# mmailhos/vectorlite

Measured on AMD Instinct MI355X. Metric: flat-cosine QPS @ N=10M dim=384 k=10; achieved HBM GB/s vs peak, higher is better.
Workload: dtype f32; 1 GPU; flat cosine single-query search, N=10000000, dim=384, k=10; rows=10000000, dim=384, k=10, metric=cosine, parallelism=1 GPU

## Files before the change

### vectorlite_amd/csrc/device_common.hpp

```cpp
#pragma once

#include <hip/hip_runtime.h>
#include <math.h>
#include <stdint.h>

#include "kernels.hpp"

namespace vl {
namespace dev {

typedef float f32x4 __attribute__((ext_vector_type(4)));

constexpr int WAVE = 64;

__device__ __forceinline__ int lane_id() { return threadIdx.x & (WAVE - 1); }

template <typename K>
__device__ __forceinline__ bool better(K ka, uint32_t pa, K kb, uint32_t pb)
{
    return ka > kb || (ka == kb && pa < pb);
}

__device__ __forceinline__ int wave_shr1_dw(int v) { return __builtin_amdgcn_update_dpp(v, v, 0x138, 0xF, 0xF, false); }
__device__ __forceinline__ float wave_shr1(float v) { return __int_as_float(wave_shr1_dw(__float_as_int(v))); }
// ... 99 lines not shown
    return rust_as_u64(__longlong_as_double((long long)key));
}


template <typename K>
__device__ __forceinline__ K neg_inf();
template <>
__device__ __forceinline__ float neg_inf<float>() { return -INFINITY; }
template <>
__device__ __forceinline__ double neg_inf<double>() { return -(double)INFINITY; }

template <typename K>
struct TopList {
    K key;
    uint32_t pos;
    K thr_key;
    uint32_t thr_pos;

    __device__ __forceinline__ void init()
    {
        key = neg_inf<K>();
        pos = POS_SENTINEL;
        asm volatile("" : "+v"(key));
        thr_key = read_lane(key, WAVE - 1);
        thr_pos = POS_SENTINEL;
    }

    __device__ __forceinline__ void insert(K k, uint32_t p)
    {
        const unsigned long long ahead = __ballot(better<K>(key, pos, k, p));
        const int idx = __popcll(ahead);
        const K upk = wave_shr1(key);
        const uint32_t upp = wave_shr1(pos);
        const int lane = lane_id();
        if (lane == idx) {
            key = k;
            pos = p;
        } else if (lane > idx) {
            key = upk;
            pos = upp;
        }
        thr_key = read_lane(key, WAVE - 1);
        thr_pos = read_lane(pos, WAVE - 1);
    }

    __device__ __forceinline__ void offer(K k, uint32_t p, bool active)
    {
        unsigned long long m = __ballot(active && better<K>(k, p, thr_key, thr_pos));
        while (m) {
            const int src = __builtin_amdgcn_readfirstlane(__ffsll((long long)m) - 1);
            m &= m - 1;
            insert(read_lane(k, src), read_lane(p, src));
        }
    }

    __device__ __forceinline__ void merge_reversed(K ok, uint32_t op)
    {
        if (better<K>(ok, op, key, pos)) {
            key = ok;
            pos = op;
        }
        const int lane = lane_id();
#pragma unroll
        for (int o = WAVE / 2; o >= 1; o >>= 1) {
            const K k2 = __shfl_xor(key, o);
            const uint32_t p2 = __shfl_xor(pos, o);
            const bool lower = (lane & o) == 0;
            const bool other_better = better<K>(k2, p2, key, pos);
            if (lower == other_better) {
                key = k2;
                pos = p2;
            }
        }
        thr_key = read_lane(key, WAVE - 1);
        thr_pos = read_lane(pos, WAVE - 1);
    }
};

template <typename K>
__device__ __forceinline__ void sort64_reversed(K& key, uint32_t& pos)
{
    const int lane = lane_id();
#pragma unroll
    for (int k = 2; k <= WAVE; k <<= 1) {
#pragma unroll
        for (int j = k >> 1; j >= 1; j >>= 1) {
            const K k2 = __shfl_xor(key, j);
            const uint32_t p2 = __shfl_xor(pos, j);
            const bool up = (lane & k) == 0;
            const bool keep_worse = ((lane & j) == 0) == up;
            const bool other_worse = better<K>(key, pos, k2, p2);
            if (keep_worse == other_worse) {
                key = k2;
                pos = p2;
            }
        }
    }
}

template <typename K, typename C, int NW>
__device__ __forceinline__ void block_merge(TopList<K>& L, C* sh )
{
    const int lane = lane_id();
    const int wave = threadIdx.x >> 6;
    sh[wave * WAVE + lane].key = L.key;
    sh[wave * WAVE + lane].pos = L.pos;
    __syncthreads();
#pragma unroll
    for (int s = NW / 2; s >= 1; s >>= 1) {
        if (wave < s) {
            const C o = sh[(wave + s) * WAVE + (WAVE - 1 - lane)];
            L.merge_reversed(o.key, o.pos);
            sh[wave * WAVE + lane].key = L.key;
            sh[wave * WAVE + lane].pos = L.pos;
        }
        __syncthreads();
    }
}

template <typename K, typename C>
__device__ __forceinline__ void block_merge_n(TopList<K>& L, C* sh, int active)
{
    const int lane = lane_id();
    const int wave = threadIdx.x >> 6;
    int top = 1;
    while (top < active) top <<= 1;
    if (wave < top) {
        sh[wave * WAVE + lane].key = L.key;
        sh[wave * WAVE + lane].pos = L.pos;
    }
    __syncthreads();
    for (int s = top / 2; s >= 1; s >>= 1) {
        if (wave < s) {
            const C o = sh[(wave + s) * WAVE + (WAVE - 1 - lane)];
            L.merge_reversed(o.key, o.pos);
            sh[wave * WAVE + lane].key = L.key;
            sh[wave * WAVE + lane].pos = L.pos;
        }
        __syncthreads();
    }
}

template <typename C>
__device__ __forceinline__ void fold_lists4_load(C (&e)[4], const C* __restrict__ lists, int first, int count)
{
    const int lane = lane_id();
#pragma unroll
    for (int i = 0; i < 4; ++i) {
        const int li = first + (i < count ? i : 0);
        const int slot = i == 0 ? lane : (KP - 1 - lane);
        if (count > 0) e[i] = lists[(size_t)li * KP + slot];
    }
}
template <typename K, typename C>
__device__ __forceinline__ void fold_lists4_merge(TopList<K>& L, const C (&e)[4], int count)
{
    L.init();
    if (count > 0) {
        L.key = e[0].key;
        L.pos = e[0].pos;
    }
#pragma unroll
    for (int i = 1; i < 4; ++i)
        if (i < count) L.merge_reversed(e[i].key, e[i].pos);
    L.thr_key = read_lane(L.key, WAVE - 1);
    L.thr_pos = read_lane(L.pos, WAVE - 1);
}
template <typename K, typename C>
__device__ __forceinline__ void fold_lists4(TopList<K>& L, const C* __restrict__ lists, int first, int count)
{
    C e[4];
    fold_lists4_load<C>(e, lists, first, count);
    fold_lists4_merge<K, C>(L, e, count);
}


}
}
```

### vectorlite_amd/csrc/kernels.hip

```cpp
#include "kernels.hpp"
#include "device_common.hpp"
#include "scan_stream.hpp"
#include "score_bound.hpp"

#include <math.h>
#include <stdlib.h>
#include <string.h>

#include <mutex>
#include <tuple>
#include <type_traits>

namespace vl {
using namespace dev;
static_assert(BOUND_COSINE == COSINE && BOUND_EUCLIDEAN == EUCLIDEAN && BOUND_MANHATTAN == MANHATTAN && BOUND_DOT == DOT,
              "score_bound.hpp carries the metric codes of kernels.hpp");
namespace {

template <typename K, typename C>
__global__ __launch_bounds__(1024) void k_merge_lists(const C* __restrict__ lists, int n_lists, size_t in_stride_q,
                                                      C* __restrict__ out, size_t out_stride_q)
{
    constexpr int NW = 16;
    __shared__ C sh[NW * WAVE];
// ... 601 lines not shown
                if (lane < n_rows) {
                    const double* t = (wave == 0) ? &S.tA[lane][0] : &S.tB[METRIC == COSINE ? lane : 0][0];
                    uint32_t cc = 0;
                    for (; cc + 16 <= cw; cc += 16) {
                        double v[16];
#pragma unroll
                        for (int u = 0; u < 16; ++u) v[u] = t[cc + u];
#pragma unroll
                        for (int u = 0; u < 16; ++u) acc += v[u];
                    }
                    for (; cc < cw; ++cc) acc += t[cc];
                }
            } else if (METRIC == COSINE && wave == 2) {
                const double* t = &S.qq[p * RP_CH];
                uint32_t cc = 0;
                for (; cc + 16 <= cw; cc += 16) {
                    double v[16];
#pragma unroll
                    for (int u = 0; u < 16; ++u) v[u] = t[cc + u];
#pragma unroll
                    for (int u = 0; u < 16; ++u) acc += v[u];
                }
                for (; cc < cw; ++cc) acc += t[cc];
            }
            if (p == 0) VL_STAMP(6);
        }
    }
    VL_STAMP(7);
    __syncthreads();
    if (METRIC == COSINE) {
        if (wave == 1 && lane < ROWS) S.b[lane] = acc;
        if (wave == 2 && lane == 0) S.c = acc;
        __syncthreads();
        if (wave == 0) {
            A.a = acc;
            A.b = S.b[lane < ROWS ? lane : 0];
            A.c = S.c;
        }
    } else if (wave == 0) {
        A.a = acc;
    }
}


template <int METRIC>
__device__ __forceinline__ void rank_check_emit(double sc, uint32_t my_pos, float key64, int n_cand, uint32_t k, uint64_t n_rows,
                                                uint32_t ld, double R, double Q, double in_extra,
                                                SearchResultBlock* __restrict__ out, uint32_t seq, const ShardRecordSink& sink,
                                                uint32_t q_in_launch)
{
    const int lane = lane_id();
    const bool valid = lane < n_cand;
    const bool any_nan = __ballot(valid && sc != sc) != 0ull;
    int rank = 0;
    for (int j = 0; j < n_cand; ++j) {
        const double sj = read_lane(sc, j);
        const uint32_t pj = read_lane(my_pos, j);
        rank += (sj > sc || (sj == sc && pj < my_pos)) ? 1 : 0;
    }
    const uint32_t k_eff = (uint64_t)k < n_rows ? k : (uint32_t)n_rows;
    uint32_t flags = 0;
    if (any_nan) flags |= RESULT_HAS_NAN | RESULT_NEEDS_EXACT;
    if (n_rows <= (uint64_t)KP) {
        if ((uint64_t)n_cand < n_rows) flags |= RESULT_NEEDS_EXACT;
    } else {
        if (n_cand < KP) {
            flags |= RESULT_NEEDS_EXACT;
        } else {
            const double B = bound_for_key<METRIC>(key64, ld, R, Q, in_extra);
            const unsigned long long at_cut = __ballot(valid && rank == (int)k_eff - 1);
            double s_cut = 0.0;
            if (at_cut) s_cut = __shfl(sc, __ffsll((long long)at_cut) - 1);
            if (!at_cut || !(s_cut > B)) flags |= RESULT_NEEDS_EXACT;
        }
    }
    if (valid && rank < (int)k_eff) {
        out->pos[rank] = my_pos;
        out->score[rank] = sc;
    }
    if (lane == 0) {
        out->n_out = k_eff;
        out->flags = flags;
    }
    if (sink.cnt) {
        const uint32_t q = sink.q0 + q_in_launch;
        const uint32_t offered = (flags == 0u) ? (k_eff < sink.ks ? k_eff : sink.ks) : 0u;
        if (valid && (uint32_t)rank < offered) {
            const size_t e = (size_t)q * sink.ks + (uint32_t)rank;
            sink.score_bits[e] = (unsigned long long)__double_as_longlong(sc);
            sink.gpos[e] = sink.row_offset + (unsigned long long)my_pos;
            sink.ids[e] = sink.pos_to_id[my_pos];
        }
        if (lane == 0) sink.cnt[q] = offered;
    }
    VL_STAMP(9);
    if (seq) {
        __threadfence_system();
        if (lane == 0) __hip_atomic_store(&out->seq, seq, __ATOMIC_RELEASE, __HIP_MEMORY_SCOPE_SYSTEM);
    }
    VL_STAMP(10);
}

constexpr int BF_ROWS = 16;
#ifndef VL_BF_NCH
#define VL_BF_NCH 4
#endif
constexpr int BF_NCH = VL_BF_NCH;
template <int METRIC>
__global__ __launch_bounds__(256) void k_batch_rescore(const Cand32* __restrict__ lists, const double* __restrict__ master,
                                                       const double* __restrict__ q64, uint32_t dim, double* __restrict__ scores)
{
    const uint32_t q = blockIdx.x >> 2, quarter = blockIdx.x & 3u;
    __shared__ RescoreLds<METRIC, BF_ROWS, BF_NCH> rs;
    __shared__ uint32_t sh_pos[BF_ROWS];
    __shared__ int sh_n;
    const int tid = threadIdx.x, lane = tid & (WAVE - 1), wave = tid >> 6;
    const Cand32* mine = lists + (size_t)q * KP + quarter * BF_ROWS;
    q64 += (size_t)q * dim;
    constexpr int QN = (RP_CH * BF_NCH + 255) / 256;
    double q_first[QN];
#pragma unroll
    for (int j = 0; j < QN; ++j) {
        const uint32_t c = (uint32_t)(tid + j * 256);
        q_first[j] = q64[c < dim ? c : dim - 1];
    }
    if (wave == 0) {
        const uint32_t p = lane < BF_ROWS ? mine[lane].pos : POS_SENTINEL;
        if (lane < BF_ROWS) sh_pos[lane] = p;
        const unsigned long long real = __ballot(p != POS_SENTINEL);
        if (lane == 0) sh_n = __popcll(real);
    }
    __syncthreads();
    const int n_mine = sh_n;
    Acc64<METRIC> A;
    rescore_rows_par<METRIC, BF_ROWS, 256, BF_NCH>(master, q64, dim, sh_pos, n_mine, rs, A, q_first);
    if (wave == 0 && lane < BF_ROWS) scores[(size_t)q * KP + quarter * BF_ROWS + lane] = lane < n_mine ? A.score() : 0.0;
}

template <int METRIC>
__global__ __launch_bounds__(256) void k_batch_rank_emit(const Cand32* __restrict__ lists, const double* __restrict__ scores,
                                                         const double* __restrict__ q_norms, uint32_t nq, uint32_t ld,
                                                         uint64_t n_rows, uint32_t k, double R, double in_extra,
                                                         SearchResultBlock* __restrict__ out, ShardRecordSink sink)
{
    const int lane = lane_id();
    const uint32_t q = blockIdx.x * 4 + (threadIdx.x >> 6);
    if (q >= nq) return;
    const Cand32 e = lists[(size_t)q * KP + lane];
    const int n_cand = __popcll(__ballot(e.pos != POS_SENTINEL));
    const double sc = lane < n_cand ? scores[(size_t)q * KP + lane] : 0.0;
    rank_check_emit<METRIC>(sc, e.pos, read_lane(e.key, KP - 1), n_cand, k, n_rows, ld, R, q_norms[q], in_extra, out + q, 0u, sink, q);
}

template <int METRIC>
__global__ __launch_bounds__(1024) void k_merge_finalize(const Cand32* __restrict__ partials, int n_lists,
                                                         size_t list_stride_q, const double* __restrict__ master,
                                                         const double* __restrict__ q64,
                                                         const double* __restrict__ q_norms, uint32_t dim,
                                                         uint32_t ld, uint64_t n_rows, uint32_t k, double R,
                                                         double in_extra, SearchResultBlock* __restrict__ out,
                                                         uint32_t seq, ShardRecordSink sink)
{
    partials += (size_t)blockIdx.x * list_stride_q;
    q64 += (size_t)blockIdx.x * dim;
    out += blockIdx.x;
    const double Q = q_norms[blockIdx.x];
    constexpr int NW = 16;
    __shared__ Cand32 sh_lists[NW * WAVE];
    __shared__ RescoreLds<METRIC> rs;
    __shared__ uint32_t sh_pos[KP];
    __shared__ float sh_key[KP];
    __shared__ int sh_ncand;

    const int lane = lane_id();
    const int wave = threadIdx.x >> 6;

    VL_STAMP(0);
    TopList<float> L;
    double q_first[1] = {0.0};
    {
        const int first = wave * 4;
        int count = n_lists - first;
        count = count < 0 ? 0 : (count > 4 ? 4 : count);
        Cand32 e[4];
        fold_lists4_load<Cand32>(e, partials, first, count);
        if (threadIdx.x < RP_BW) q_first[0] = q64[threadIdx.x < dim ? threadIdx.x : dim - 1];
        fold_lists4_merge<float, Cand32>(L, e, count);
    }
    VL_STAMP(1);
    block_merge_n<float, Cand32>(L, sh_lists, (n_lists + 3) / 4);
    VL_STAMP(2);
    if (wave == 0) {
        sh_pos[lane] = L.pos;
        sh_key[lane] = L.key;
        const unsigned long long real = __ballot(L.pos != POS_SENTINEL);
        if (lane == 0) sh_ncand = __popcll(real);
    }
    __syncthreads();
    const int n_cand = sh_ncand;

    Acc64<METRIC> A;
    VL_STAMP(3);
    rescore_rows_par<METRIC, KP, 1024>(master, q64, dim, sh_pos, n_cand, rs, A, q_first);
    VL_STAMP(8);

    if (wave == 0) {
        const bool valid = lane < n_cand;
        const double sc = valid ? A.score() : 0.0;
        rank_check_emit<METRIC>(sc, sh_pos[lane], sh_key[KP - 1], n_cand, k, n_rows, ld, R, Q, in_extra, out, seq, sink, blockIdx.x);
    }
}

constexpr int KMULTI_PARTS = 4;

template <int METRIC>
__global__ __launch_bounds__(1024) void k_merge_finalize_multi(const Cand32* __restrict__ lists, int n_lists,
                                                               size_t part_stride, int n_parts,
                                                               const double* __restrict__ master,
                                                               const double* __restrict__ q64,
                                                               const double* __restrict__ q_norms, uint32_t dim,
                                                               uint32_t ld, uint64_t n_rows, uint32_t k, double R,
                                                               SearchResultBlock* __restrict__ out)
{
    constexpr int NW = 16;
    __shared__ Cand32 sh_lists[NW * WAVE];
    __shared__ RescoreLds<METRIC> rs;
    __shared__ uint32_t sh_pos[KMULTI_PARTS * KP];
    __shared__ float sh_key[KMULTI_PARTS * KP];
    __shared__ double sh_score[KMULTI_PARTS * KP];
    __shared__ int sh_ncand[KMULTI_PARTS];
    __shared__ int sh_flags;
    __shared__ double sh_cut;
    __shared__ int sh_has_cut;
    const double Q = q_norms[0];
    const int lane = lane_id();
    const int wave = threadIdx.x >> 6;
    double q_first[1] = {0.0};
    if (threadIdx.x < RP_BW) q_first[0] = q64[threadIdx.x < dim ? threadIdx.x : dim - 1];
    if (threadIdx.x == 0) {
        sh_flags = 0;
        sh_has_cut = 0;
        sh_cut = 0.0;
    }
    for (int p = 0; p < n_parts; ++p) {
        TopList<float> L;
        const int first = wave * 4;
        int count = n_lists - first;
        count = count < 0 ? 0 : (count > 4 ? 4 : count);
        fold_lists4<float, Cand32>(L, lists + (size_t)p * part_stride, first, count);
        block_merge<float, Cand32, NW>(L, sh_lists);
        if (wave == 0) {
            sh_pos[p * KP + lane] = L.pos;
            sh_key[p * KP + lane] = L.key;
            const unsigned long long real = __ballot(L.pos != POS_SENTINEL);
            if (lane == 0) sh_ncand[p] = __popcll(real);
        }
        __syncthreads();
    }
    for (int p = 0; p < n_parts; ++p) {
        Acc64<METRIC> A;
        rescore_rows_par<METRIC, KP, 1024>(master, q64, dim, sh_pos + p * KP, sh_ncand[p], rs, A, q_first);
        if (wave == 0) sh_score[p * KP + lane] = lane < sh_ncand[p] ? A.score() : 0.0;
        __syncthreads();
    }
    const int t = threadIdx.x;
    const int total_slots = n_parts * KP;
    const bool valid = t < total_slots && (t % KP) < sh_ncand[t / KP];
    const double sc = valid ? sh_score[t] : 0.0;
    const uint32_t my_pos = t < total_slots ? sh_pos[t] : POS_SENTINEL;
    if (valid && sc != sc) atomicOr(&sh_flags, (int)(RESULT_HAS_NAN | RESULT_NEEDS_EXACT));
    int rank = 0;
    for (int j = 0; j < total_slots; ++j) {
        if ((j % KP) >= sh_ncand[j / KP]) continue;
        const double sj = sh_score[j];
        const uint32_t pj = sh_pos[j];
        rank += (sj > sc || (sj == sc && pj < my_pos)) ? 1 : 0;
    }
    const uint32_t k_eff = (uint64_t)k < n_rows ? k : (uint32_t)n_rows;
    if (valid && rank == (int)k_eff - 1) {
        sh_cut = sc;
        sh_has_cut = 1;
    }
    __syncthreads();
    if (valid && rank < (int)k_eff) {
        out[rank / KP].pos[rank % KP] = my_pos;
        out[rank / KP].score[rank % KP] = sc;
    }
    if (t == 0) {
        uint32_t flags = (uint32_t)sh_flags;
        int total = 0;
        double B = -1.0e300;
        bool excluded_rows = false;
        for (int p = 0; p < n_parts; ++p) {
            total += sh_ncand[p];
            if (sh_ncand[p] == KP) {
                excluded_rows = true;
                const double bp = bound_for_key<METRIC>(sh_key[p * KP + KP - 1], ld, R, Q, 0.0);
                B = bp > B ? bp : B;
            }
        }
        if (!sh_has_cut || (uint32_t)total < k_eff) flags |= RESULT_NEEDS_EXACT;
        else if (excluded_rows && !(sh_cut > B)) flags |= RESULT_NEEDS_EXACT;
        if ((uint64_t)total < n_rows && !excluded_rows) flags |= RESULT_NEEDS_EXACT;
        out[0].n_out = k_eff;
        out[0].flags = flags;
    }
}

constexpr int EX_ROWS = 256;
constexpr int EX_CH = 16;

template <int METRIC>
__global__ __launch_bounds__(256) void k_exact_scan(const double* __restrict__ master,
                                                    const double* __restrict__ q64, uint64_t n, uint32_t dim,
                                                    double* __restrict__ scores, uint32_t* __restrict__ nan_flag)
{
    __shared__ double tile[EX_ROWS][EX_CH + 1];
    __shared__ double qtile[EX_CH];
    const int tid = threadIdx.x;
    const uint64_t n_tiles = (n + EX_ROWS - 1) / EX_ROWS;
    const uint32_t n_chunks = (dim + EX_CH - 1) / EX_CH;
    for (uint64_t t = blockIdx.x; t < n_tiles; t += gridDim.x) {
        const uint64_t row0 = t * EX_ROWS;
        const uint64_t rows_here = (n - row0) < (uint64_t)EX_ROWS ? (n - row0) : (uint64_t)EX_ROWS;
        Acc64<METRIC> A;
        A.init();
        double pre[EX_CH];
        double qpre = 0.0;
        auto fetch = [&](uint32_t c0) {
            const uint32_t cw = (dim - c0) < (uint32_t)EX_CH ? (dim - c0) : (uint32_t)EX_CH;
#pragma unroll
            for (int i = 0; i < EX_CH; ++i) {
                const int idx = tid + i * 256;
                uint64_t r = (uint64_t)(idx / EX_CH);
                uint32_t cc = (uint32_t)(idx % EX_CH);
                r = r < rows_here ? r : rows_here - 1;
                cc = cc < cw ? cc : cw - 1;
                pre[i] = master[(row0 + r) * dim + c0 + cc];
            }
            {
                uint32_t qc = (uint32_t)(tid % EX_CH);
                qc = qc < cw ? qc : cw - 1;
                qpre = q64[c0 + qc];
// ... 830 lines not shown
                if (qarg) {                                                                                 \
                    ScanQArg qa;                                                                            \
                    memcpy(qa.v, q32_host, (size_t)ld * sizeof(float));                                     \
                    launch(Fam::template qarg<G, VPL, U>(), std::make_tuple(n32), std::make_tuple(qa));     \
                    launched = true;                                                                        \
                }                                                                                           \
            }                                                                                               \
            if constexpr (Fam::Q64_AT_ANY_STRIDE || G * VPL * 4 > SCAN_QARG_FLOATS) {                       \
                if (!launched) {                                                                            \
                    launch(Fam::template q64<G, VPL, U>(), std::make_tuple(q64, dim, n32), std::tuple<>()); \
                    launched = true;                                                                        \
                }                                                                                           \
            }                                                                                               \
        }                                                                                                   \
    }
        VL_SCAN_VARIANTS(VL_TRY_VARIANT)
#undef VL_TRY_VARIANT
        if (!launched) return hipErrorInvalidValue;
    } else {
#define VL_SCAN_GEN(G) \
    case G: launch(Fam::template generic<G>(), std::make_tuple(q64, dim, n32, ld4), std::tuple<>()); break;
        switch (sh.g) {
            VL_SCAN_GEN(1)
            VL_SCAN_GEN(2)
            VL_SCAN_GEN(4)
            VL_SCAN_GEN(8)
            VL_SCAN_GEN(16)
            VL_SCAN_GEN(32)
            VL_SCAN_GEN(64)
        default: return hipErrorInvalidValue;
        }
#undef VL_SCAN_GEN
    }
    return hipGetLastError();
}
}

bool scan_takes_qarg(uint32_t ld)
{
    if ((ld & 3) || ld > (uint32_t)SCAN_QARG_FLOATS) return false;
    return default_scan_shape(ld / 4).special;
}

hipError_t launch_scan(hipStream_t s, int metric, const float* slab, const float* inv_norm, const double* q64,
                       uint64_t n, uint32_t dim, uint32_t ld, Cand32* partials, ScanPlan* plan, const float* q32_host)
{
    if (n == 0 || n >= 0xFFFFFFFFull || (ld & 3)) return hipErrorInvalidValue;
    const ScanShape sh = scan_shape(ld / 4);
    const f32x4* slab4 = reinterpret_cast<const f32x4*>(slab);
    if (!shape_takes_qarg(sh, ld, q32_host) && !q64) return hipErrorInvalidValue;
    int grid = 0;
    hipError_t rc = dispatch_metric(metric, [&](auto M) -> hipError_t {
        return launch_scan_family<TopFamily<decltype(M)::value>>(s, sh, n, ld, q64, dim, q32_host,
                                                                 std::make_tuple(slab4, inv_norm), std::make_tuple(partials), &grid);
    });
    if (plan) {
        plan->grid = grid;
        plan->variant = sh.special ? (sh.g * 10000 + sh.vpl * 100 + sh.u) : -sh.g;
    }
    return rc;
}

#define VL_BATCH_SHAPES(X) X(4, 2) X(4, 4) X(8, 1) X(8, 2) X(8, 3) X(8, 4) X(8, 6) X(8, 8) X(8, 10) X(8, 12) X(8, 16) X(16, 10) X(16, 12) X(16, 16) X(16, 24)

bool scan_batch_supported(uint32_t ld)
{
    const uint32_t ld4 = ld / 4;
    bool ok = false;
#define VL_CHK(G, VPL) ok = ok || ((uint32_t)(G * VPL) == ld4);
    VL_BATCH_SHAPES(VL_CHK)
#undef VL_CHK
    return ok && (ld % 4) == 0;
}

hipError_t launch_scan_batch(hipStream_t s, int metric, const float* slab, const float* inv_norm, const double* q64,
                             uint32_t nq, uint64_t n, uint32_t dim, uint32_t ld, Cand32* partials, ScanPlan* plan)
{
    if (n == 0 || n >= 0xFFFFFFFFull || (ld & 3) || nq == 0 || nq > (uint32_t)SCAN_BATCH_MAX_QUERIES) return hipErrorInvalidValue;
    const uint32_t ld4 = ld / 4;
    const f32x4* slab4 = reinterpret_cast<const f32x4*>(slab);
    const uint32_t n32 = (uint32_t)n;
    const uint32_t groups = (nq + SCAN_BATCH_QB - 1) / SCAN_BATCH_QB;
    int grid = 0;
    hipError_t rc = dispatch_metric(metric, [&](auto M) -> hipError_t {
        constexpr int MM = decltype(M)::value;
        bool launched = false;
#define VL_TRY_BATCH(G, VPL)                                                                                  \
    if (!launched && (uint32_t)(G * VPL) == ld4) {                                                            \
        auto kern = k_scan_batch<MM, G, VPL, SCAN_BATCH_QB>;                                                  \
        int cus = 0;                                                                                          \
        const int resident = resident_blocks(reinterpret_cast<const void*>(kern), &cus);                      \
        const uint64_t steps = (n + (64 / G) - 1) / (64 / G);                                                 \
        uint64_t blocks = (steps + 3) / 4;                                                                    \
        uint64_t cap = (uint64_t)env_int("VL_BATCH_GRID", 0);                                                 \
        if (cap == 0) cap = (uint64_t)resident;                                                               \
        if (cap > (uint64_t)SCAN_BATCH_MAX_GRID) cap = SCAN_BATCH_MAX_GRID;                                   \
        if (groups > 1) {                                                                                     \
             \
              \
            cap = std::max<uint64_t>(1, cap / groups);                                                        \
            cap = std::min<uint64_t>(cap, 64);                                                                \
            cap = std::min<uint64_t>(cap, std::max<uint64_t>(1, PARTIALS32_LISTS / ((uint64_t)groups * SCAN_BATCH_QB))); \
        }                                                                                                     \
        if (blocks > cap) blocks = cap;                                                                       \
        grid = (int)(blocks < 1 ? 1 : blocks);                                                                \
        hipLaunchKernelGGL(kern, dim3(grid, groups), dim3(256), 0, s, slab4, inv_norm, q64, nq, dim, n32, partials); \
        launched = true;                                                                                      \
    }
        VL_BATCH_SHAPES(VL_TRY_BATCH)
#undef VL_TRY_BATCH
        if (!launched) return hipErrorInvalidValue;
        return hipGetLastError();
    });
    if (plan) {
        plan->grid = grid;
        plan->variant = 0;
    }
    return rc;
}

namespace {
template <typename K, typename C>
const C* reduce_lists(hipStream_t s, const C* lists, int* n_lists, size_t* stride_q, int nq, C* scratch)
{
    int n = *n_lists;
    size_t in_stride = *stride_q;
    int ping = 0;
    while (n > 64) {
        const int blocks = (n + 63) / 64;
        const size_t out_stride = (size_t)64 * KP;
        C* out = scratch + (size_t)ping * nq * out_stride;
        hipLaunchKernelGGL((k_merge_lists<K, C>), dim3(blocks, nq), dim3(1024), 0, s, lists, n, in_stride, out,
                           out_stride);
        lists = out;
        in_stride = out_stride;
        n = blocks;
        ping ^= 1;
    }
    *n_lists = n;
    *stride_q = in_stride;
    return lists;
}
}

hipError_t launch_merge_finalize(hipStream_t s, int metric, Cand32* partials, int n_lists, int nq,
                                 const double* master, const double* q64, const double* q_norms, uint32_t dim,
                                 uint64_t n_rows, uint32_t k, double max_row_norm, SearchResultBlock* out,
                                 double in_extra, uint32_t seq, const ShardRecordSink* sink)
{
    if (seq && nq != 1) return hipErrorInvalidValue;
    const ShardRecordSink sk = sink ? *sink : ShardRecordSink{};
    const uint32_t ld = (dim + 3u) & ~3u;
    size_t stride = (size_t)n_lists * KP;
    const Cand32* lists = reduce_lists<float, Cand32>(s, partials, &n_lists, &stride, nq, partials + PARTIALS32_LISTS * KP);
    return dispatch_metric(metric, [&](auto M) -> hipError_t {
        constexpr int MM = decltype(M)::value;
        hipLaunchKernelGGL((k_merge_finalize<MM>), dim3(nq), dim3(1024), 0, s, lists, n_lists, stride, master, q64,
                           q_norms, dim, ld, n_rows, k, max_row_norm, in_extra, out, seq, sk);
        return hipGetLastError();
    });
}

hipError_t launch_batch_finalize(hipStream_t s, int metric, const Cand32* lists, int nq, const double* master, const double* q64,
                                 const double* q_norms, uint32_t dim, uint64_t n_rows, uint32_t k, double max_row_norm,
                                 SearchResultBlock* out, double in_extra, double* score_scratch, const ShardRecordSink* sink)
{
    if (nq <= 0 || !score_scratch) return hipErrorInvalidValue;
    const uint32_t ld = (dim + 3u) & ~3u;
    const ShardRecordSink sk = sink ? *sink : ShardRecordSink{};
    return dispatch_metric(metric, [&](auto M) -> hipError_t {
        constexpr int MM = decltype(M)::value;
        hipLaunchKernelGGL((k_batch_rescore<MM>), dim3((unsigned)nq * 4u), dim3(256), 0, s, lists, master, q64, dim, score_scratch);
        hipLaunchKernelGGL((k_batch_rank_emit<MM>), dim3(((unsigned)nq + 3u) / 4u), dim3(256), 0, s, lists, (const double*)score_scratch,
                           q_norms, (uint32_t)nq, ld, n_rows, k, max_row_norm, in_extra, out, sk);
        return hipGetLastError();
    });
}

hipError_t launch_merge_finalize_multi(hipStream_t s, int metric, Cand32* partials, int n_lists_total, int n_parts,
                                       const double* master, const double* q64, const double* q_norm, uint32_t dim,
                                       uint64_t n_rows, uint32_t k, double max_row_norm, SearchResultBlock* out)
{
    if (n_parts < 2 || n_parts > KMULTI_PARTS || n_lists_total % n_parts != 0) return hipErrorInvalidValue;
    const uint32_t ld = (dim + 3u) & ~3u;
    int n_lists = n_lists_total / n_parts;
    size_t stride = (size_t)n_lists * KP;
    const Cand32* lists = reduce_lists<float, Cand32>(s, partials, &n_lists, &stride, n_parts, partials + PARTIALS32_LISTS * KP);
    return dispatch_metric(metric, [&](auto M) -> hipError_t {
        constexpr int MM = decltype(M)::value;
        hipLaunchKernelGGL((k_merge_finalize_multi<MM>), dim3(1), dim3(1024), 0, s, lists, n_lists, stride, n_parts, master,
                           q64, q_norm, dim, ld, n_rows, k, max_row_norm, out);
        return hipGetLastError();
    });
}

hipError_t launch_exact_scan(hipStream_t s, int metric, const double* master, const double* q64, uint64_t n,
                             uint32_t dim, double* scores, uint32_t* nan_flag)
{
    if (n == 0) return hipSuccess;
    const uint64_t tiles = (n + EX_ROWS - 1) / EX_ROWS;
    const int grid = (int)(tiles < 4096 ? tiles : 4096);
    return dispatch_metric(metric, [&](auto M) -> hipError_t {
        constexpr int MM = decltype(M)::value;
        hipLaunchKernelGGL((k_exact_scan<MM>), dim3(grid), dim3(256), 0, s, master, q64, n, dim, scores, nan_flag);
        return hipGetLastError();
    });
}

hipError_t launch_exact_scan_subset(hipStream_t s, int metric, const double* master, const double* q64, const uint32_t* plist,
                                    uint64_t m, uint32_t dim, double* scores, uint32_t* nan_flag)
{
    if (m == 0) return hipSuccess;
    const uint64_t tiles = (m + EX_ROWS - 1) / EX_ROWS;
    const int grid = (int)(tiles < 4096 ? tiles : 4096);
    return dispatch_metric(metric, [&](auto M) -> hipError_t {
        constexpr int MM = decltype(M)::value;
        hipLaunchKernelGGL((k_exact_scan_subset<MM>), dim3(grid), dim3(256), 0, s, master, q64, plist, m, dim, scores, nan_flag);
        return hipGetLastError();
    });
}

bool scan_subset_takes_qarg(uint32_t ld) { return scan_takes_qarg(ld); }

hipError_t launch_scan_subset(hipStream_t s, int metric, const float* slab, const float* inv_norm, const uint32_t* plist,
                              uint64_t m, const double* q64, uint32_t dim, uint32_t ld, Cand32* partials, ScanPlan* plan,
                              const float* q32_host)
{
    if (m == 0 || m >= 0xFFFFFFFFull || (ld & 3)) return hipErrorInvalidValue;
    const ScanShape sh = default_scan_shape(ld / 4);
    const f32x4* slab4 = reinterpret_cast<const f32x4*>(slab);
    if (!shape_takes_qarg(sh, ld, q32_host) && !q64) return hipErrorInvalidValue;
    int grid = 0;
    hipError_t rc = dispatch_metric(metric, [&](auto M) -> hipError_t {
        return launch_scan_family<SubsetFamily<decltype(M)::value>>(s, sh, m, ld, q64, dim, q32_host,
                                                                    std::make_tuple(slab4, inv_norm, plist),
                                                                    std::make_tuple(partials), &grid);
    });
    if (plan) {
        plan->grid = grid;
        plan->variant = sh.special ? (SUBSET_VARIANT_BASE + sh.g * 10000 + sh.vpl * 100 + sh.u) : -(SUBSET_VARIANT_BASE + sh.g);
    }
    return rc;
}

int filter_grid_for(uint64_t n, uint32_t* chunk)
{
    uint64_t c = (n + FILTER_MAX_GRID - 1) / FILTER_MAX_GRID;
    if (c < 1024) c = 1024;
    *chunk = (uint32_t)c;
    return (int)((n + c - 1) / c);
}

hipError_t launch_filter_count(hipStream_t s, const unsigned long long* pos_ids, uint64_t n, const unsigned long long* fids,
                               uint64_t nf, uint32_t* counts, uint32_t* m_out)
{
    if (n == 0 || n >= 0xFFFFFFFFull || nf == 0 || nf >= 0xFFFFFFFFull) return hipErrorInvalidValue;
    uint32_t chunk = 0;
    const int grid = filter_grid_for(n, &chunk);
    hipLaunchKernelGGL(k_filter_count, dim3(grid), dim3(256), 0, s, pos_ids, (uint32_t)n, fids, (uint32_t)nf, chunk, counts);
    hipLaunchKernelGGL(k_filter_scan, dim3(1), dim3(FILTER_MAX_GRID), 0, s, counts, (uint32_t)grid, m_out);
    return hipGetLastError();
}

hipError_t launch_filter_compact(hipStream_t s, const unsigned long long* pos_ids, uint64_t n, const unsigned long long* fids,
                                 uint64_t nf, const uint32_t* offsets, uint64_t m, uint32_t* plist)
{
    if (n == 0 || n >= 0xFFFFFFFFull || nf == 0 || nf >= 0xFFFFFFFFull || m == 0) return hipErrorInvalidValue;
    uint32_t chunk = 0;
    const int grid = filter_grid_for(n, &chunk);
    hipLaunchKernelGGL(k_filter_compact, dim3(grid), dim3(256), 0, s, pos_ids, (uint32_t)n, fids, (uint32_t)nf, chunk, offsets,
                       (uint32_t)m, plist);
    return hipGetLastError();
}

int select_grid_for(uint64_t n)
{
    const uint64_t steps = (n + 63) / 64;
    uint64_t blocks = (steps + 3) / 4;
    if (blocks > (uint64_t)SELECT_MAX_GRID) blocks = SELECT_MAX_GRID;
    if (blocks < 1) blocks = 1;
    return (int)blocks;
}

hipError_t launch_exact_select(hipStream_t s, const double* scores, uint64_t n, uint32_t k, Cand64* partials,
                               const uint32_t* nan_flag, SearchResultBlock* out, const SearchResultBlock* after)
{
    if (n == 0 || n >= 0xFFFFFFFFull || k > (uint32_t)KP) return hipErrorInvalidValue;
    const int grid = select_grid_for(n);
    hipLaunchKernelGGL(k_select64, dim3(grid), dim3(256), 0, s, scores, (uint32_t)n, after, partials);
    hipError_t e = hipGetLastError();
    if (e != hipSuccess) return e;
    int n_lists = grid;
    size_t stride = (size_t)n_lists * KP;
    const Cand64* lists = reduce_lists<double, Cand64>(s, partials, &n_lists, &stride, 1, partials + (size_t)SELECT_MAX_GRID * KP);
    hipLaunchKernelGGL(k_merge64_emit, dim3(1), dim3(1024), 0, s, lists, n_lists, n, k, nan_flag, out);
    return hipGetLastError();
}

uint64_t sort_capacity_for(uint64_t n)
{
    uint64_t cap = SORT_LOCAL;
    while (cap < n) cap <<= 1;
    return cap;
}

namespace {
template <typename P>
// ... 162 lines not shown
```

### vectorlite_amd/csrc/kernels.hpp

```cpp
#pragma once

#include <hip/hip_runtime.h>
#include <stddef.h>
#include <stdint.h>

namespace vl {

enum Metric : int { COSINE = 0, EUCLIDEAN = 1, MANHATTAN = 2, DOT = 3 };

constexpr int KP = 64;
constexpr int KFAST_MAX = 60;
constexpr uint32_t POS_SENTINEL = 0xFFFFFFFFu;

struct Cand32 {
    float key;
    uint32_t pos;
};
struct Cand64 {
    double key;
    uint32_t pos;
    uint32_t pad;
};

struct SearchResultBlock {
    uint32_t n_out;
    uint32_t flags;
    uint32_t pos[KP];
    double score[KP];
    uint32_t seq;
    uint32_t pad;
};
constexpr uint32_t RESULT_NEEDS_EXACT = 1u;
constexpr uint32_t RESULT_HAS_NAN = 2u;

struct ShardRecordSink {
    unsigned long long* cnt = nullptr;
    unsigned long long* score_bits = nullptr;
    unsigned long long* gpos = nullptr;
    unsigned long long* ids = nullptr;
    const unsigned long long* pos_to_id = nullptr;
    unsigned long long row_offset = 0;
    uint32_t ks = 0;
    uint32_t q0 = 0;
};

struct IngestStats {
    unsigned long long max_norm_bits;
    unsigned int n_out_of_domain;
    unsigned int pad;
};

constexpr uint8_t ROW_OUT_OF_DOMAIN = 1;

struct ScanPlan {
    int grid;
    int variant;
};

hipError_t launch_embed_f32(hipStream_t s, const float* emb, uint64_t n, uint32_t dim, bool normalize, double* out);

hipError_t launch_ingest(hipStream_t s, const double* master, float* slab, float* inv_norm, uint8_t* flags,
                         IngestStats* stats, uint64_t n, uint32_t dim, uint32_t ld);

constexpr int SCAN_MAX_GRID = 4096;
constexpr int SELECT_MAX_GRID = 1024;
constexpr int SCAN_BATCH_QB = 8;
constexpr int SCAN_BATCH_MAX_GRID = 2048;
constexpr int SCAN_BATCH_MAX_QUERIES = 512;
constexpr size_t PARTIALS32_LISTS = (size_t)SCAN_BATCH_QB * SCAN_BATCH_MAX_GRID;
static_assert(PARTIALS32_LISTS >= (size_t)SCAN_MAX_GRID, "single-query lists must fit");
constexpr size_t PARTIALS32_ENTRIES = (PARTIALS32_LISTS + 2 * (size_t)SCAN_BATCH_QB * 64) * KP;
constexpr size_t PARTIALS64_ENTRIES = (size_t)(SELECT_MAX_GRID + 128) * KP;

constexpr int SCAN_QARG_FLOATS = 768;
bool scan_takes_qarg(uint32_t ld);
hipError_t launch_scan(hipStream_t s, int metric, const float* slab, const float* inv_norm, const double* q64,
                       uint64_t n, uint32_t dim, uint32_t ld, Cand32* partials, ScanPlan* plan,
                       const float* q32_host = nullptr);

constexpr int KMULTI_MAX = 220;
hipError_t launch_merge_finalize_multi(hipStream_t s, int metric, Cand32* partials, int n_lists_total, int n_parts,
                                       const double* master, const double* q64, const double* q_norm, uint32_t dim,
                                       uint64_t n_rows, uint32_t k, double max_row_norm, SearchResultBlock* out);
hipError_t launch_merge_finalize(hipStream_t s, int metric, Cand32* partials, int n_lists, int nq,
                                 const double* master, const double* q64, const double* q_norms, uint32_t dim,
                                 uint64_t n_rows, uint32_t k, double max_row_norm, SearchResultBlock* out,
                                 double in_extra = 0.0, uint32_t seq = 0, const ShardRecordSink* sink = nullptr);
inline hipError_t launch_merge_finalize(hipStream_t s, uint32_t seq, int metric, Cand32* partials, int n_lists,
                                        const double* master, const double* q64, const double* q_norm, uint32_t dim,
                                        uint64_t n_rows, uint32_t k, double max_row_norm, SearchResultBlock* out,
                                        double in_extra)
{
    return launch_merge_finalize(s, metric, partials, n_lists, 1, master, q64, q_norm, dim, n_rows, k, max_row_norm, out,
                                 in_extra, seq);
}

hipError_t launch_batch_finalize(hipStream_t s, int metric, const Cand32* lists, int nq, const double* master, const double* q64,
                                 const double* q_norms, uint32_t dim, uint64_t n_rows, uint32_t k, double max_row_norm,
                                 SearchResultBlock* out, double in_extra, double* score_scratch,
                                 const ShardRecordSink* sink = nullptr);

bool scan_batch_supported(uint32_t ld);
hipError_t launch_scan_batch(hipStream_t s, int metric, const float* slab, const float* inv_norm, const double* q64,
                             uint32_t nq, uint64_t n, uint32_t dim, uint32_t ld, Cand32* partials, ScanPlan* plan);

hipError_t launch_exact_scan(hipStream_t s, int metric, const double* master, const double* q64, uint64_t n,
                             uint32_t dim, double* scores, uint32_t* nan_flag);
constexpr int SUBSET_VARIANT_BASE = 3000000;
bool scan_subset_takes_qarg(uint32_t ld);
hipError_t launch_scan_subset(hipStream_t s, int metric, const float* slab, const float* inv_norm, const uint32_t* plist,
                              uint64_t m, const double* q64, uint32_t dim, uint32_t ld, Cand32* partials, ScanPlan* plan,
                              const float* q32_host = nullptr);
hipError_t launch_exact_scan_subset(hipStream_t s, int metric, const double* master, const double* q64, const uint32_t* plist,
                                    uint64_t m, uint32_t dim, double* scores, uint32_t* nan_flag);
constexpr int FILTER_COUNTS_MAX = 1024;
hipError_t launch_filter_count(hipStream_t s, const unsigned long long* pos_ids, uint64_t n, const unsigned long long* fids,
                               uint64_t nf, uint32_t* counts, uint32_t* m_out);
hipError_t launch_filter_compact(hipStream_t s, const unsigned long long* pos_ids, uint64_t n, const unsigned long long* fids,
                                 uint64_t nf, const uint32_t* offsets, uint64_t m, uint32_t* plist);

constexpr int RANGE_VARIANT_BASE = 4000000;
constexpr uint32_t RANGE_CAND_MAX = 1u << 20;
constexpr uint32_t RANGE_SMALL = 2048;
constexpr int RANGE_CTR_APPENDED = 0, RANGE_CTR_TOTAL = 1, RANGE_CTR_NAN = 2, RANGE_CTR_GROUP_NAN = 3, RANGE_CTR_WORDS = 4;
bool scan_range_takes_qarg(uint32_t ld);
hipError_t launch_scan_range(hipStream_t s, int metric, const float* slab, const float* inv_norm, const uint32_t* plist,
                             uint64_t n, const double* q64, uint32_t dim, uint32_t ld, float tau, uint32_t* cand,
                             uint32_t cap, uint32_t* ctr, ScanPlan* plan, const float* q32_host = nullptr);
hipError_t launch_range_rescore(hipStream_t s, int metric, const double* master, const double* q64, const uint32_t* cand,
                                uint32_t cap, uint32_t dim, double* scores, uint32_t* ctr);
hipError_t launch_range_cut(hipStream_t s, const double* scores, const uint32_t* cand, const uint32_t* m_ptr, uint64_t m_max,
                            double min_score, uint64_t* keys, uint64_t* pv, uint64_t store_cap, uint32_t* ctr,
                            const uint32_t* group_of_row = nullptr, uint64_t n_rows = 0, bool keep_nan = false);
hipError_t launch_range_rank(hipStream_t s, uint64_t* keys, uint64_t* pv, const double* scores, const uint32_t* total_ptr,
                             uint64_t total, uint64_t k, uint32_t* out_pos, double* out_scores);

hipError_t launch_group_rows(hipStream_t s, const unsigned long long* pos_ids, uint64_t n, const unsigned long long* fids,
                             const uint32_t* dense, uint64_t nf, uint32_t* group_of_row);
constexpr int GROUP_VARIANT_BASE = 5000000;
constexpr uint32_t GROUPED_MAX_K = 1024;
hipError_t launch_scan_group_best(hipStream_t s, int metric, const float* slab, const float* inv_norm, const uint32_t* plist,
                                  uint64_t n, const double* q64, uint32_t dim, uint32_t ld, const uint32_t* group_of_row,
                                  uint64_t* best, ScanPlan* plan, const float* q32_host = nullptr);
constexpr int GROUP_TOP_LISTS = 64;
hipError_t launch_group_top(hipStream_t s, const uint64_t* best, uint64_t n_groups, uint32_t k, Cand32* lists, uint32_t* cand,
                            uint32_t* ctr);
hipError_t launch_group_collapse(hipStream_t s, const uint64_t* pv, const double* scores, const uint32_t* n_ptr, uint64_t n_max,
                                 const uint32_t* group_of_row, uint64_t n_rows, const uint64_t* group_keys, uint64_t n_groups,
                                 uint32_t* first, uint32_t k, uint64_t* out_keys, uint32_t* out_pos, double* out_scores,
                                 uint32_t* out_n);

constexpr uint32_t RBATCH_SEG = 2048;
constexpr int RBATCH_CTR_TOTAL = 0, RBATCH_CTR_NAN = 1, RBATCH_CTR_OFF = 2, RBATCH_CTR_WANT = 3, RBATCH_CTR_WORDS = 4;
hipError_t launch_range_batch_tail(hipStream_t s, int metric, const Cand32* cand, const uint32_t* cnt, uint32_t cap, uint32_t nq,
                                   const double* master, const double* q64, const double* min_scores, uint32_t dim,
                                   uint64_t n_rows, uint32_t emit_cap, double* sv_score, uint32_t* sv_pos, uint32_t* ctr,
                                   uint32_t* out_pos, double* out_scores);

int select_grid_for(uint64_t n);
hipError_t launch_exact_select(hipStream_t s, const double* scores, uint64_t n, uint32_t k, Cand64* partials,
                               const uint32_t* nan_flag, SearchResultBlock* out,
                               const SearchResultBlock* after = nullptr);
constexpr int SELECT_MAX_ROUNDS = 16;
uint64_t sort_capacity_for(uint64_t n);
hipError_t launch_exact_sort(hipStream_t s, const double* scores, uint64_t n, uint64_t k, uint64_t* okeys,
                             uint32_t* opos, uint32_t* out_pos, double* out_scores);

constexpr uint32_t MMR_MAX_FETCH = 1024;
struct MmrSource {
    const SearchResultBlock* blocks = nullptr;
    const uint32_t* pos = nullptr;
    const double* scores = nullptr;
    const uint32_t* plist = nullptr;
    const uint32_t* nan_flag = nullptr;
    uint32_t plist_len = 0;
    uint32_t n = 0;
    uint32_t n_block0 = 0;
    uint32_t n_rows = 0;
};
hipError_t launch_mmr(hipStream_t s, int metric, const double* master, uint32_t dim, const MmrSource& src, double* sim,
                      uint32_t k, double lambda, SearchResultBlock* out, uint32_t seq);

hipError_t launch_hnsw_distances(hipStream_t s, int metric, const double* master, const double* q64,
                                 uint32_t dim, const uint32_t* positions, uint32_t m, uint64_t* out);

}
```

Measured before the change: 1583 queries/s.

## Merge partial top-k lists inside finalize kernel via prefix threshold selection

For single-query search with up to 1024 partial lists, the separate reduce_lists merge passes are skipped and the finalize kernel merges the partials itself. Each thread reads the first 8 entries of one list, a block-wide threshold prunes the candidates, and if at most 256 survive they are sorted and merged directly. Otherwise it falls back to picking the 64 lists whose heads rank in the top 64 and folding only those. This removes extra kernel launches and intermediate memory traffic, at the cost of more complex in-kernel logic and extra synchronisation.

```diff
diff --git a/vectorlite_amd/csrc/device_common.hpp b/vectorlite_amd/csrc/device_common.hpp
--- a/vectorlite_amd/csrc/device_common.hpp
+++ b/vectorlite_amd/csrc/device_common.hpp
@@ -275,6 +275,16 @@
         if (count > 0) e[i] = lists[(size_t)li * KP + slot];
     }
 }
+template <typename C>
+__device__ __forceinline__ void fold_lists4_load(C (&e)[4], const C* __restrict__ lists, const int* sel, int first, int count)
+{
+    const int lane = lane_id();
+#pragma unroll
+    for (int i = 0; i < 4; ++i) {
+        const int slot = i == 0 ? lane : (KP - 1 - lane);
+        if (count > 0) e[i] = lists[(size_t)sel[first + (i < count ? i : 0)] * KP + slot];
+    }
+}
 template <typename K, typename C>
 __device__ __forceinline__ void fold_lists4_merge(TopList<K>& L, const C (&e)[4], int count)
 {
diff --git a/vectorlite_amd/csrc/kernels.hip b/vectorlite_amd/csrc/kernels.hip
--- a/vectorlite_amd/csrc/kernels.hip
+++ b/vectorlite_amd/csrc/kernels.hip
@@ -777,6 +777,99 @@
     rank_check_emit<METRIC>(sc, e.pos, read_lane(e.key, KP - 1), n_cand, k, n_rows, ld, R, q_norms[q], in_extra, out + q, 0u, sink, q);
 }
 
+constexpr int SEL_PRE = 8;
+constexpr int SEL_CAND_MAX = 256;
+
+__device__ __forceinline__ bool merge_prefixes(const Cand32 (&pre)[SEL_PRE], TopList<float>& L, Cand32* sh, int* wave_cnt,
+                                               float* wave_thr)
+{
+    const int lane = lane_id();
+    const int wave = threadIdx.x >> 6;
+    float s = pre[0].key;
+#pragma unroll
+    for (int k = 2; k <= WAVE; k <<= 1) {
+#pragma unroll
+        for (int j = k >> 1; j >= 1; j >>= 1) {
+            const float o = __shfl_xor(s, j);
+            const bool keep_min = ((lane & j) == 0) == ((lane & k) == 0);
+            s = keep_min ? fminf(s, o) : fmaxf(s, o);
+        }
+    }
+    const float fourth = read_lane(s, WAVE - 4);
+    if (lane == 0) wave_thr[wave] = fourth;
+    __syncthreads();
+    float t = wave_thr[0];
+#pragma unroll
+    for (int w = 1; w < 16; ++w) t = fminf(t, wave_thr[w]);
+    int c = 0;
+#pragma unroll
+    for (int i = 0; i < SEL_PRE; ++i) c += (pre[i].pos != POS_SENTINEL && pre[i].key >= t) ? 1 : 0;
+    int incl = c;
+#pragma unroll
+    for (int o = 1; o < WAVE; o <<= 1) {
+        const int y = __shfl_up(incl, o);
+        if (lane >= o) incl += y;
+    }
+    if (lane == WAVE - 1) wave_cnt[wave] = incl;
+    const int overflow = __syncthreads_or(c == SEL_PRE ? 1 : 0);
+    int base = 0, total = 0;
+#pragma unroll
+    for (int w = 0; w < 16; ++w) {
+        const int n = wave_cnt[w];
+        base += w < wave ? n : 0;
+        total += n;
+    }
+    if (overflow || total > SEL_CAND_MAX) return false;
+    const int slot = base + incl - c;
+#pragma unroll
+    for (int i = 0; i < SEL_PRE; ++i)
+        if (i < c) sh[slot + i] = pre[i];
+    __syncthreads();
+    const int n_sorts = (total + WAVE - 1) / WAVE;
+    L.init();
+    if (wave < n_sorts) {
+        const int idx = wave * WAVE + lane;
+        Cand32 e = sh[idx < total ? idx : 0];
+        if (idx >= total) {
+            e.key = neg_inf<float>();
+            e.pos = POS_SENTINEL;
+        }
+        sort64_reversed<float>(e.key, e.pos);
+        L.key = __shfl(e.key, WAVE - 1 - lane);
+        L.pos = __shfl(e.pos, WAVE - 1 - lane);
+    }
+    block_merge_n<float, Cand32>(L, sh, n_sorts);
+    return true;
+}
+
+__device__ __forceinline__ int select_lists64(float hk, uint32_t hp, int li, Cand32* sh, int* sel, int* wave_cnt)
+{
+    const int lane = lane_id();
+    const int wave = threadIdx.x >> 6;
+    TopList<float> H;
+    float sk = hk;
+    uint32_t sp = hp;
+    sort64_reversed<float>(sk, sp);
+    H.key = __shfl(sk, WAVE - 1 - lane);
+    H.pos = __shfl(sp, WAVE - 1 - lane);
+    block_merge_n<float, Cand32>(H, sh, 16);
+    const Cand32 T = sh[KP - 1];
+    const bool take = hp != POS_SENTINEL && !better<float>(T.key, T.pos, hk, hp);
+    const unsigned long long m = __ballot(take);
+    if (lane == 0) wave_cnt[wave] = __popcll(m);
+    __syncthreads();
+    int base = 0, total = 0;
+    for (int w = 0; w < 16; ++w) {
+        const int c = wave_cnt[w];
+        base += w < wave ? c : 0;
+        total += c;
+    }
+    const int slot = base + __popcll(m & ((1ull << lane) - 1ull));
+    if (take && slot < KP) sel[slot] = li;
+    __syncthreads();
+    return total < KP ? total : KP;
+}
+
 template <int METRIC>
 __global__ __launch_bounds__(1024) void k_merge_finalize(const Cand32* __restrict__ partials, int n_lists,
                                                          size_t list_stride_q, const double* __restrict__ master,
@@ -796,6 +889,9 @@
     __shared__ uint32_t sh_pos[KP];
     __shared__ float sh_key[KP];
     __shared__ int sh_ncand;
+    __shared__ int sh_sel[KP];
+    __shared__ int sh_wave_cnt[NW];
+    __shared__ float sh_wave_thr[NW];
 
     const int lane = lane_id();
     const int wave = threadIdx.x >> 6;
@@ -803,17 +899,44 @@
     VL_STAMP(0);
     TopList<float> L;
     double q_first[1] = {0.0};
-    {
+    const bool pick = n_lists > KP;
+    bool merged = false;
+    int n_fold = n_lists;
+    if (pick) {
+        const int li = lane * NW + wave;
+        const bool has = li < n_lists;
+        const uint4* src = reinterpret_cast<const uint4*>(partials + (size_t)(has ? li : n_lists - 1) * KP);
+        uint4 v[SEL_PRE / 2];
+#pragma unroll
+        for (int i = 0; i < SEL_PRE / 2; ++i) v[i] = src[i];
+        if (threadIdx.x < RP_BW) q_first[0] = q64[threadIdx.x < dim ? threadIdx.x : dim - 1];
+        Cand32 pre[SEL_PRE];
+#pragma unroll
+        for (int i = 0; i < SEL_PRE / 2; ++i) {
+            pre[2 * i].key = has ? __uint_as_float(v[i].x) : neg_inf<float>();
+            pre[2 * i].pos = has ? v[i].y : POS_SENTINEL;
+            pre[2 * i + 1].key = has ? __uint_as_float(v[i].z) : neg_inf<float>();
+            pre[2 * i + 1].pos = has ? v[i].w : POS_SENTINEL;
+        }
+        merged = merge_prefixes(pre, L, sh_lists, sh_wave_cnt, sh_wave_thr);
+        VL_STAMP(11);
+        if (!merged) n_fold = select_lists64(pre[0].key, pre[0].pos, li, sh_lists, sh_sel, sh_wave_cnt);
+    }
+    if (!merged) {
         const int first = wave * 4;
-        int count = n_lists - first;
+        int count = n_fold - first;
         count = count < 0 ? 0 : (count > 4 ? 4 : count);
         Cand32 e[4];
-        fold_lists4_load<Cand32>(e, partials, first, count);
-        if (threadIdx.x < RP_BW) q_first[0] = q64[threadIdx.x < dim ? threadIdx.x : dim - 1];
+        if (pick) {
+            fold_lists4_load<Cand32>(e, partials, sh_sel, first, count);
+        } else {
+            fold_lists4_load<Cand32>(e, partials, first, count);
+            if (threadIdx.x < RP_BW) q_first[0] = q64[threadIdx.x < dim ? threadIdx.x : dim - 1];
+        }
         fold_lists4_merge<float, Cand32>(L, e, count);
     }
     VL_STAMP(1);
-    block_merge_n<float, Cand32>(L, sh_lists, (n_lists + 3) / 4);
+    if (!merged) block_merge_n<float, Cand32>(L, sh_lists, (n_fold + 3) / 4);
     VL_STAMP(2);
     if (wave == 0) {
         sh_pos[lane] = L.pos;
@@ -1950,7 +2073,9 @@
     const ShardRecordSink sk = sink ? *sink : ShardRecordSink{};
     const uint32_t ld = (dim + 3u) & ~3u;
     size_t stride = (size_t)n_lists * KP;
-    const Cand32* lists = reduce_lists<float, Cand32>(s, partials, &n_lists, &stride, nq, partials + PARTIALS32_LISTS * KP);
+    const bool in_finalize = nq == 1 && n_lists <= MERGE_IN_FINALIZE_MAX_LISTS && env_int("VL_MERGE_IN_FINALIZE", 1) != 0;
+    const Cand32* lists = partials;
+    if (!in_finalize) lists = reduce_lists<float, Cand32>(s, partials, &n_lists, &stride, nq, partials + PARTIALS32_LISTS * KP);
     return dispatch_metric(metric, [&](auto M) -> hipError_t {
         constexpr int MM = decltype(M)::value;
         hipLaunchKernelGGL((k_merge_finalize<MM>), dim3(nq), dim3(1024), 0, s, lists, n_lists, stride, master, q64,
diff --git a/vectorlite_amd/csrc/kernels.hpp b/vectorlite_amd/csrc/kernels.hpp
--- a/vectorlite_amd/csrc/kernels.hpp
+++ b/vectorlite_amd/csrc/kernels.hpp
@@ -82,6 +82,7 @@
 hipError_t launch_merge_finalize_multi(hipStream_t s, int metric, Cand32* partials, int n_lists_total, int n_parts,
                                        const double* master, const double* q64, const double* q_norm, uint32_t dim,
                                        uint64_t n_rows, uint32_t k, double max_row_norm, SearchResultBlock* out);
+constexpr int MERGE_IN_FINALIZE_MAX_LISTS = 1024;
 hipError_t launch_merge_finalize(hipStream_t s, int metric, Cand32* partials, int n_lists, int nq,
                                  const double* master, const double* q64, const double* q_norms, uint32_t dim,
                                  uint64_t n_rows, uint32_t k, double max_row_norm, SearchResultBlock* out,
```

Measured after the change: 1593 queries/s (median of 5 runs). About the same (+0.6%).
